# lucaspk512/vrdone

Measured on AMD Instinct MI355X. Metric: subject-object pairs/sec forward (2048 pairs x 256 frames x 512-d), higher is better.
Workload: dtype f16x3: f32 products as 3 scaled-f16 MFMA products (~22-bit), f32 accumulate; reference-grade: distance to a float64 run of the reference <= 1.4 x the reference's own float32 error (tests/golden/mask_vrd_f64.npz)

## Files before the change

### vrdone_amd/csrc/vrd_attn_x3.hip

```cpp
#include "vrd_common.h"
#include <cmath>
#include <cstdlib>
#include <type_traits>
#include <utility>

namespace {

using f32x16 = __attribute__((ext_vector_type(16))) float;
typedef __attribute__((ext_vector_type(8))) __bf16 bf16x8;
typedef __attribute__((ext_vector_type(4))) __bf16 bf16x4;
typedef __attribute__((ext_vector_type(4))) short s16x4;
typedef __attribute__((ext_vector_type(8))) short s16x8;
typedef __attribute__((address_space(3))) void* lds_ptr_t;
typedef __attribute__((address_space(3))) s16x4* lds_s16x4_ptr;

__device__ uint4 g_attn_zero[16];

template <int HD>
struct AG {
    static constexpr int ROWB = HD * 2;
    static constexpr int CPR = ROWB / 16;
    static constexpr int RPI = 1024 / ROWB;
    static constexpr int PLANE = 32 * ROWB;
    static constexpr int STAGE = 4 * PLANE;
// ... 251 lines not shown
__device__ __forceinline__ void split_pair(float p0, float p1, unsigned& hi, unsigned& lo) {
    if constexpr (F16) {
        typedef __attribute__((ext_vector_type(2))) _Float16 f16x2;
        const f16x2 h = {(_Float16)p0, (_Float16)p1};
        hi = __builtin_bit_cast(unsigned, h);
        const f16x2 l = {(_Float16)(p0 - (float)h[0]), (_Float16)(p1 - (float)h[1])};
        lo = __builtin_bit_cast(unsigned, l);
    } else {
        const bf16x2 h = {(__bf16)p0, (__bf16)p1};
        hi = __builtin_bit_cast(unsigned, h);
        const float h0 = __builtin_bit_cast(float, hi << 16), h1 = __builtin_bit_cast(float, hi & 0xffff0000u);
        const bf16x2 l = {(__bf16)(p0 - h0), (__bf16)(p1 - h1)};
        lo = __builtin_bit_cast(unsigned, l);
    }
}

#define VRD_MFMA(pre, ops, ...)                                                   \
    do {                                                                          \
        if constexpr (F16) asm volatile(pre "v_mfma_f32_32x32x16_f16 " ops __VA_ARGS__);  \
        else asm volatile(pre "v_mfma_f32_32x32x16_bf16 " ops __VA_ARGS__);       \
    } while (0)

template <int R0, int N>
__device__ __forceinline__ void agpr_scale(float alpha) {
    if constexpr (N > 0) {
        float t;
        asm volatile("v_accvgpr_read_b32 %0, a%c2\n\tv_mul_f32 %0, %0, %1\n\tv_accvgpr_write_b32 a%c2, %0"
                     : "=&v"(t) : "v"(alpha), "n"(R0));
        agpr_scale<R0 + 1, N - 1>(alpha);
    }
}

struct SmBlock {
    float x[16];
    float mx, mu, ae, alpha, sum;
    float mr, lp;
    u32x4 ph[2], pl[2];
};

#ifdef VRD_ATTN_STAMP
__device__ unsigned long long g_attn_stamp[65];
#define VRD_STAMP(i)                                                                      \
    do {                                                                                  \
        if (wave == 0) {                                                                  \
            unsigned long long t_;                                                        \
            asm volatile("s_memtime %0\n\ts_waitcnt lgkmcnt(0)" : "=s"(t_)::"memory");    \
            if (lane == 0) stamp_lds[i] = t_;                                             \
        }                                                                                 \
    } while (0)
#else
#define VRD_STAMP(i) do { } while (0)
#endif

template <int HD, bool F16, int NPROD = 3>
__global__ __launch_bounds__(256, 1) void attn_flash_x3_w64_kernel(const float* __restrict__ q, int64_t ldq,
                                                                  const float* __restrict__ k, const float* __restrict__ v,
                                                                  int64_t ldkv, const uint8_t* __restrict__ kv_mask,
                                                                  const uint8_t* __restrict__ q_mask, int Tq, int Tk, int width,
                                                                  float scale_log2e, float* __restrict__ out, int64_t ldo,
                                                                  int pair_out, int q_blocks, int n_head_, int n_batch, int prefetch, int item_step) {
    using G = AG<HD>;
    static_assert(NPROD == 3 || (NPROD == 1 && F16), "the one-product form exists for the f16 format only");
    constexpr bool LO = NPROD == 3;
    constexpr int KS = HD / 16;
    constexpr int DT = HD / 32;
    constexpr int NS = 4;
    constexpr int PER_WAVE = G::N_DMA / 4;
    constexpr int PPP = 32 / G::RPI;
    constexpr int NG_S = 6 * KS;
    constexpr int NG_O = 12 * DT;
    constexpr int HPG_S = 48 / NG_S, HPG_O = 48 / NG_O;
    constexpr int LEAD = 4;
#define VRD_AQ(qb, s) (8 * ((qb) * KS + (s)))
#define VRD_AO(qb, d) (128 + 16 * ((qb) * DT + (d)))
    static_assert(G::N_DMA % 4 == 0 && NG_S >= 24 && NG_O >= 24 && VRD_AQ(1, KS - 1) + 8 <= 128, "layout assumptions");
    extern __shared__ __attribute__((aligned(16))) float smem[];
    char* const lds = reinterpret_cast<char*>(smem);
    const int nkt = (Tk + 31) / 32, nqg = (Tq + 31) / 32;
    float* const kbias = reinterpret_cast<float*>(lds + NS * G::STAGE);
    int* const tile_on = reinterpret_cast<int*>(kbias + nkt * 32);
    int* const qgrp = tile_on + nkt;
    const int nk64 = (nkt * 32 + 63) & ~63, nq64 = (nqg * 32 + 63) & ~63;
    int* const raw_k = qgrp + nqg;
    int* const raw_q = raw_k + nk64;
#ifdef VRD_ATTN_STAMP
    unsigned long long* const stamp_lds = reinterpret_cast<unsigned long long*>(lds + 163840 - 64 * 8);
#endif

    const int tid = threadIdx.x, lane = tid & 63;
    const int wave = __builtin_amdgcn_readfirstlane(tid >> 6);
    const int li = lane & 31, lh = lane >> 5;
    const unsigned lds_base = (unsigned)reinterpret_cast<uintptr_t>((lds_ptr_t)lds);
    const int n_items = n_head_ * n_batch;
    bool masks_pending = true;
    auto fresh_lane = [&]() {
        int ln;
        asm volatile("v_mbcnt_lo_u32_b32 %0, -1, 0\n\tv_mbcnt_hi_u32_b32 %0, -1, %0" : "=v"(ln));
        return ln;
    };
    auto dma_masks = [&](int it2) {
        const int b2 = it2 / n_head_;
        const int ln = fresh_lane();
        if (kv_mask) {
            const uint8_t* base = kv_mask + (int64_t)b2 * Tk;
            for (int j = wave; j < nk64 / 64; j += 4) {
                const int key = j * 64 + ln;
                const unsigned voff = (unsigned)(key < Tk ? key : Tk - 1);
                const unsigned dst = lds_base + (unsigned)(reinterpret_cast<char*>(raw_k) - lds) + j * 256;
                asm volatile("s_mov_b32 m0, %0\n\ts_nop 0\n\tglobal_load_lds_ubyte %1, %2" ::"s"(dst), "v"(voff), "s"(base) : "memory");
            }
        }
        if (q_mask) {
            const uint8_t* base = q_mask + (int64_t)b2 * Tq;
            for (int j = wave; j < nq64 / 64; j += 4) {
                const int r = j * 64 + ln;
                const unsigned voff = (unsigned)(r < Tq ? r : Tq - 1);
                const unsigned dst = lds_base + (unsigned)(reinterpret_cast<char*>(raw_q) - lds) + j * 256;
                asm volatile("s_mov_b32 m0, %0\n\ts_nop 0\n\tglobal_load_lds_ubyte %1, %2" ::"s"(dst), "v"(voff), "s"(base) : "memory");
            }
        }
    };
    const int item_first = item_step == 1 ? (int)(((long long)n_items * blockIdx.x) / gridDim.x) : (int)blockIdx.x;
    const int item_end = item_step == 1 ? (int)(((long long)n_items * (blockIdx.x + 1)) / gridDim.x) : n_items;
    for (int item = item_first; item < item_end; item += item_step) {
    VRD_STAMP(0);
    const int h = item % n_head_, b = item / n_head_;
    if (prefetch && item == item_first) dma_masks(item);
    if (prefetch && masks_pending) asm volatile("s_waitcnt vmcnt(0)" ::: "memory");
    asm volatile("s_waitcnt lgkmcnt(0)" ::: "memory");
    __builtin_amdgcn_s_barrier();
    asm volatile("" ::: "memory");
    {
        const int ln = fresh_lane(), tn = wave * 64 + ln;
        for (int key = tn; key < nkt * 32; key += 256) {
            const bool ok = key < Tk && (!kv_mask || (prefetch ? raw_k[key] != 0 : kv_mask[(int64_t)b * Tk + (key < Tk ? key : Tk - 1)] != 0));
            kbias[key] = ok ? 0.f : -INFINITY;
            const unsigned long long bal = __ballot(ok);
            const unsigned bits = (unsigned)((bal >> (ln & 32)) & 0xffffffffull);
            if ((ln & 31) == 0) tile_on[key >> 5] = bits == 0u ? 0 : (bits == 0xffffffffu ? 2 : 1);
        }
        for (int r = tn; r < nqg * 32; r += 256) {
            const bool ok = r < Tq && (!q_mask || (prefetch ? raw_q[r] != 0 : q_mask[(int64_t)b * Tq + (r < Tq ? r : Tq - 1)] != 0));
            const unsigned long long bal = __ballot(ok);
            if ((ln & 31) == 0) qgrp[r >> 5] = ((bal >> (ln & 32)) & 0xffffffffull) != 0ull;
        }
    }
    asm volatile("s_waitcnt lgkmcnt(0)" ::: "memory");
    __builtin_amdgcn_s_barrier();
    asm volatile("" ::: "memory");
    if (prefetch && item + item_step < item_end) {
        dma_masks(item + item_step);
        masks_pending = true;
    }
    VRD_STAMP(1);
    for (int qblk = 0; qblk < q_blocks; ++qblk) {
    if (qblk) {
        asm volatile("s_waitcnt lgkmcnt(0)" ::: "memory");
        __builtin_amdgcn_s_barrier();
        asm volatile("" ::: "memory");
    }
    const int q0 = qblk * 256 + wave * 64;
    const char* kb = reinterpret_cast<const char*>(k + (int64_t)b * Tk * ldkv) + h * HD * 4;
    const char* vb = reinterpret_cast<const char*>(v + (int64_t)b * Tk * ldkv) + h * HD * 4;

    const int gq = qblk * 8 + (lane & 7);
    const unsigned blk_bits = (unsigned)(__ballot(gq < nqg && qgrp[gq < nqg ? gq : 0] != 0) & 0xffull);
    const bool live0 = (blk_bits >> (2 * wave)) & 1u, live1 = (blk_bits >> (2 * wave + 1)) & 1u;
    const bool q_live = live0 || live1;
    if (blk_bits == 0u) {
#ifndef VRD_ATTN_LAB_NOZERO
        {
            constexpr int LPRZ = HD / 4, RPIZ = 64 / LPRZ;
            const int row_end = Tq < qblk * 256 + 256 ? Tq : qblk * 256 + 256;
            const int ln = fresh_lane();
            int row = qblk * 256 + wave * RPIZ + ln / LPRZ;
            char* zp = reinterpret_cast<char*>(out + ((int64_t)b * Tq + row) * ldo) + h * HD * 4 + (ln % LPRZ) * 16;
            const int64_t zstep = ldo * 4 * (4 * RPIZ);
            const u32x4 zero4 = {0u, 0u, 0u, 0u};
#pragma unroll 1
            for (; row < row_end; row += 4 * RPIZ, zp += zstep) *reinterpret_cast<u32x4*>(zp) = zero4;
        }
#endif
        continue;
    }
    VRD_STAMP(55);
    asm volatile("" ::: VRD_ALL_AGPRS);
    {
        const char* qbase = reinterpret_cast<const char*>(q + (int64_t)b * Tq * ldq) + h * HD * 4;
        const int rin_q = lane / G::CPR, pch_q = lane % G::CPR;
        const unsigned qrowbytes = (unsigned)(ldq * 4);
        static_for<2 * PPP>([&](auto u_c) {
            constexpr int qb = decltype(u_c)::value / PPP, rb = decltype(u_c)::value % PPP;
            const int row = rb * G::RPI + rin_q;
            const int tq = q0 + 32 * qb + row;
            const int lc = pch_q ^ G::kswz(row);
            const unsigned voff = (unsigned)(tq < Tq ? tq : Tq - 1) * qrowbytes + (unsigned)((lc >> 2) * 128 + (lc & 3) * 16);
            const unsigned dst = lds_base + (2 * qb + (wave >> 1)) * G::STAGE + (wave & 1) * 2 * G::PLANE + rb * 1024;
            const char* const src_hi = qbase + 0;
            const char* const src_lo = src_hi + 64;
            asm volatile("s_mov_b32 m0, %0\n\ts_nop 0\n\tglobal_load_lds_dwordx4 %1, %2" ::"s"(dst), "v"(voff), "s"(src_hi) : "memory");
            asm volatile("s_mov_b32 m0, %0\n\ts_nop 0\n\tglobal_load_lds_dwordx4 %1, %2" ::"s"(dst + G::PLANE), "v"(voff), "s"(src_lo) : "memory");
        });
    }
    VRD_STAMP(56);
    static_for<2 * DT * 16>([&](auto r_c) {
        asm volatile("v_accvgpr_write_b32 a%c0, 0" :: "n"(128 + decltype(r_c)::value));
    });
    VRD_STAMP(57);

    const int rin = lane / G::CPR, pch = lane % G::CPR;
    const int row0 = (wave % PPP) * G::RPI + rin;
    const int rowbytes = (int)(ldkv * 4);
    auto chunk_of = [&](int row, bool is_v) {
        const int lc = pch ^ (is_v ? G::vswz(row) : G::kswz(row));
        return (lc >> 2) * 128 + (lc & 3) * 16;
    };
    constexpr int HALF_ROWS = HD == 128 ? 16 : 0;
    struct Req {
        const char *kbase, *vbase;
        unsigned vk[2], vv[2];
        int half;
    };
    auto req_of = [&](int kt) {
        Req r;
        if (kt * 32 + 32 <= Tk) {
            r.kbase = kb + (int64_t)kt * 32 * rowbytes;
            r.vbase = vb + (int64_t)kt * 32 * rowbytes;
            r.vk[0] = r.vk[1] = (unsigned)(row0 * rowbytes) + chunk_of(row0, false);
            r.vv[0] = r.vv[1] = (unsigned)(row0 * rowbytes) + chunk_of(row0, true);
            r.half = HALF_ROWS * rowbytes;
        } else {
            r.kbase = kb;
            r.vbase = vb;
#pragma unroll
            for (int u = 0; u < 2; ++u) {
                int key = kt * 32 + row0 + HALF_ROWS * u;
                key = key < Tk ? key : Tk - 1;
                r.vk[u] = (unsigned)(key * rowbytes) + chunk_of(row0, false);
                r.vv[u] = (unsigned)(key * rowbytes) + chunk_of(row0, true);
            }
            r.half = 0;
        }
        return r;
    };
    auto issue1 = [&](const Req& r, int buf, auto i_c) __attribute__((always_inline)) {
        constexpr int i = decltype(i_c)::value;
        constexpr int u = HD == 128 ? (i & 1) : 0;
        const int j = wave + 4 * i;
        const int plane = j / PPP, rb = j % PPP;
        const unsigned dst = lds_base + buf * G::STAGE + plane * G::PLANE + rb * 1024;
        const char* sbase = (plane < 2 ? r.kbase : r.vbase) + ((plane & 1) ? 64 : 0) + (u ? r.half : 0);
        const unsigned voff = plane < 2 ? r.vk[u] : r.vv[u];
        asm volatile("s_mov_b32 m0, %0\n\ts_nop 0\n\tglobal_load_lds_dwordx4 %1, %2" ::"s"(dst), "v"(voff), "s"(sbase) : "memory");
    };

    unsigned long long act = ~0ull;
    if (nkt <= 64) act = __ballot(lane < nkt && tile_on[lane < nkt ? lane : 0] != 0);
    auto next_on = [&](int from) {
        if (from >= nkt) return nkt;
        if (nkt > 64) return from;
        const unsigned long long m = act & (~0ull << from);
        return m ? (int)__builtin_ctzll(m) : nkt;
    };
    const int n_act = nkt <= 64 ? (int)__builtin_popcountll(act) : nkt;
    unsigned long long cln = 0ull;
    if (nkt <= 64) cln = __ballot(lane < nkt && tile_on[lane < nkt ? lane : 0] == 2);
    const int krow = li * G::ROWB;
    const int vq = (lane >> 2) & 3, vp = lane & 3;
    const int vcol0 = 16 * ((lane >> 4) & 1) + 4 * vp;

    struct KF { bf16x8 h, l; };
    auto load_k = [&](const char* st, int s) __attribute__((always_inline)) {
        KF f;
        const int off = krow + (((2 * s + lh) ^ G::kswz(li)) * 16);
        f.h = *reinterpret_cast<const bf16x8*>(st + off);
        if (LO) f.l = *reinterpret_cast<const bf16x8*>(st + G::PLANE + off);
        return f;
    };
    auto load_v = [&](const char* st, int s, int d) __attribute__((always_inline)) {
        KF f;
        s16x8 rh, rl;
#pragma unroll
        for (int part = 0; part < 2; ++part) {
            const int row = 16 * s + 8 * part + 4 * lh + vq;
            const int col = 32 * d + vcol0;
            const int off = row * G::ROWB + ((((col * 2) >> 4) ^ G::vswz(row)) * 16) + ((col * 2) & 15);
            const s16x4 th = __builtin_amdgcn_ds_read_tr16_b64_v4i16((lds_s16x4_ptr)(st + 2 * G::PLANE + off));
            s16x4 tl = th;
            if (LO) tl = __builtin_amdgcn_ds_read_tr16_b64_v4i16((lds_s16x4_ptr)(st + 3 * G::PLANE + off));
#pragma unroll
            for (int j = 0; j < 4; ++j) {
                rh[4 * part + j] = th[j];
                rl[4 * part + j] = tl[j];
            }
        }
        f.h = __builtin_bit_cast(bf16x8, rh);
        f.l = __builtin_bit_cast(bf16x8, rl);
        return f;
    };

    SmBlock A, B;
    A.mr = B.mr = -INFINITY;
    A.lp = B.lp = 0.f;
    float tsp[4];
    unsigned long long cmask[2] = {0ull, 0ull};
    const float thr = F16 ? 8.0f : 16.0f;
// ... 100 lines not shown
        } else if constexpr (i == 72) {
            float ta, tb;
            asm volatile("v_exp_f32 %2, %6\n\tv_exp_f32 %3, %7\n\tv_add_f32 %4, %8, %10\n\tv_add_f32 %5, %9, %11\n\t"
                         "v_fma_f32 %0, %0, %2, %4\n\tv_fma_f32 %1, %1, %3, %5"
                         : "+v"(A.lp), "+v"(B.lp), "=&v"(A.alpha), "=&v"(B.alpha), "=&v"(ta), "=&v"(tb)
                         : "v"(A.ae), "v"(B.ae), "v"(A.sum), "v"(B.sum), "v"(A.x[15]), "v"(B.x[15]));
        }
    };

    auto mfma_s = [&](auto s_c, auto j_c, const KF& kf, f32x16& sa, f32x16& sb) __attribute__((always_inline)) {
        constexpr int s = decltype(s_c)::value, j = decltype(j_c)::value, qb = j & 1;
        f32x16& acc = qb ? sb : sa;
        constexpr int aq = VRD_AQ(qb, s) + (j >= 2 && j < 4 ? 4 : 0);
        if constexpr (!LO) {
            if constexpr (j < 4) {
            } else if constexpr (s == 0)
                VRD_MFMA("", "%0, %1, a[%c2:%c3], 0", : "=&v"(acc) : "v"(kf.h), "n"(aq), "n"(aq + 3));
            else
                VRD_MFMA("", "%0, %1, a[%c2:%c3], %0", : "+v"(acc) : "v"(kf.h), "n"(aq), "n"(aq + 3));
        } else if constexpr (s == 0 && j < 2) {
            VRD_MFMA("", "%0, %1, a[%c2:%c3], 0", : "=&v"(acc) : "v"(kf.l), "n"(aq), "n"(aq + 3));
        } else if constexpr (j < 2) {
            VRD_MFMA("", "%0, %1, a[%c2:%c3], %0", : "+v"(acc) : "v"(kf.l), "n"(aq), "n"(aq + 3));
        } else {
            VRD_MFMA("", "%0, %1, a[%c2:%c3], %0", : "+v"(acc) : "v"(kf.h), "n"(aq), "n"(aq + 3));
        }
    };
    auto mfma_o = [&](auto g_c, auto j_c, const KF& vf) __attribute__((always_inline)) {
        constexpr int g = decltype(g_c)::value, j = decltype(j_c)::value, qb = j & 1, s = g / DT, d = g % DT;
        constexpr int ao = VRD_AO(qb, d);
        const SmBlock& X = qb ? B : A;
        if constexpr (!LO) {
            if constexpr (j < 4) {
            } else if constexpr (d == 0 && j == 4)
                VRD_MFMA("s_nop 1\n\t", "a[%c2:%c3], %0, %1, a[%c2:%c3]", :: "v"(vf.h), "v"(X.ph[s]), "n"(ao), "n"(ao + 15));
            else
                VRD_MFMA("", "a[%c2:%c3], %0, %1, a[%c2:%c3]", :: "v"(vf.h), "v"(X.ph[s]), "n"(ao), "n"(ao + 15));
        } else if constexpr (j < 2) {
            if constexpr (d == 0 && j == 0)
                VRD_MFMA("s_nop 1\n\t", "a[%c2:%c3], %0, %1, a[%c2:%c3]", :: "v"(vf.l), "v"(X.ph[s]), "n"(ao), "n"(ao + 15));
            else
                VRD_MFMA("", "a[%c2:%c3], %0, %1, a[%c2:%c3]", :: "v"(vf.l), "v"(X.ph[s]), "n"(ao), "n"(ao + 15));
        } else if constexpr (j < 4) {
            VRD_MFMA("", "a[%c2:%c3], %0, %1, a[%c2:%c3]", :: "v"(vf.h), "v"(X.pl[s]), "n"(ao), "n"(ao + 15));
        } else {
            VRD_MFMA("", "a[%c2:%c3], %0, %1, a[%c2:%c3]", :: "v"(vf.h), "v"(X.ph[s]), "n"(ao), "n"(ao + 15));
        }
    };
    auto rescale = [&](auto qb_c, float alpha) __attribute__((always_inline)) {
        agpr_scale<VRD_AO(decltype(qb_c)::value, 0), 16 * DT>(alpha);
    };

    auto tile = [&](auto with_s_c, f32x16& sa_c, f32x16& sb_c, f32x16& sa_n, f32x16& sb_n, const char* st,
                    const char* st1, const float* kbs, bool dirty, bool do_req, const Req& req, int buf_req, bool first) __attribute__((always_inline)) {
        constexpr bool WITH_S = decltype(with_s_c)::value;
        if (dirty) {
#pragma unroll
            for (int g = 0; g < 4; ++g) {
                const float4 bv = *reinterpret_cast<const float4*>(kbs + 8 * g + 4 * lh);
                sa_c[4 * g + 0] += bv.x;
                sa_c[4 * g + 1] += bv.y;
                sa_c[4 * g + 2] += bv.z;
                sa_c[4 * g + 3] += bv.w;
                sb_c[4 * g + 0] += bv.x;
                sb_c[4 * g + 1] += bv.y;
                sb_c[4 * g + 2] += bv.z;
                sb_c[4 * g + 3] += bv.w;
            }
        }
        KF kf{}, kn{}, vf{}, vn{};
        if (WITH_S) kf = load_k(st1, 0);
        VRD_SB();
        static_for<LEAD>([&](auto u_c) { sm_piece(u_c, sa_c, sb_c); });
        VRD_SB();
        static_for<KS>([&](auto s_c) {
            constexpr int s = decltype(s_c)::value;
            static_for<6>([&](auto j_c) {
                constexpr int j = decltype(j_c)::value, gap = 6 * s + j;
                if constexpr (WITH_S) mfma_s(s_c, j_c, kf, sa_n, sb_n);
                if constexpr (j == 0 && WITH_S && s + 1 < KS) kn = load_k(st1, s + 1);
                if constexpr (gap == NG_S - 4) vf = load_v(st, 0, 0);
                static_for<HPG_S>([&](auto u_c) {
                    constexpr int piece = LEAD + gap * HPG_S + decltype(u_c)::value;
                    if constexpr (piece < 48) sm_piece(ic<piece>{}, sa_c, sb_c);
                });
                VRD_SB();
            });
            kf = kn;
        });
        if (!first && cmask[0] != 0ull) rescale(ic<0>{}, __builtin_amdgcn_exp2f(A.ae));
        if (!first && cmask[1] != 0ull) rescale(ic<1>{}, __builtin_amdgcn_exp2f(B.ae));
        VRD_SB();
        static_for<2 * DT>([&](auto g_c) {
            constexpr int g = decltype(g_c)::value;
            static_for<6>([&](auto j_c) {
                constexpr int j = decltype(j_c)::value, gap = 6 * g + j;
                mfma_o(g_c, j_c, vf);
                if constexpr (j == 0 && g + 1 < 2 * DT) vn = load_v(st, (g + 1) / DT, (g + 1) % DT);
                static_for<HPG_O>([&](auto u_c) { sm_piece(ic<48 + gap * HPG_O + decltype(u_c)::value>{}, sa_c, sb_c); });
                constexpr int rq = gap - NG_O / 2 - 1;
                if constexpr (rq >= 0 && rq % 3 == 0 && rq / 3 < PER_WAVE) {
                    if (do_req) issue1(req, buf_req, ic<rq / 3>{});
                }
                VRD_SB();
            });
            vf = vn;
        });
    };

    int kt_iss = -1;
    int issued = 0;
    auto request_next = [&](int buf) {
        if (issued < n_act) {
            kt_iss = next_on(kt_iss + 1);
            const Req r = req_of(kt_iss);
            static_for<PER_WAVE>([&](auto i_c) { issue1(r, buf, i_c); });
            ++issued;
        }
    };
    VRD_STAMP(51);
    asm volatile("s_waitcnt vmcnt(0)" ::: "memory");
    masks_pending = false;
    VRD_STAMP(52);
    static_for<2>([&](auto qb_c) {
        constexpr int qb = decltype(qb_c)::value;
        static_for<KS>([&](auto s_c) {
            constexpr int s = decltype(s_c)::value;
            const char* stq = lds + (2 * qb + (wave >> 1)) * G::STAGE + (wave & 1) * 2 * G::PLANE;
            const int off = li * G::ROWB + (((2 * s + lh) ^ G::kswz(li)) * 16);
            const u32x4 th = *reinterpret_cast<const u32x4*>(stq + off), tl = *reinterpret_cast<const u32x4*>(stq + G::PLANE + off);
            constexpr int r = VRD_AQ(qb, s);
            asm volatile("v_accvgpr_write_b32 a%c8, %0\n\tv_accvgpr_write_b32 a%c9, %1\n\tv_accvgpr_write_b32 a%c10, %2\n\t"
                         "v_accvgpr_write_b32 a%c11, %3\n\tv_accvgpr_write_b32 a%c12, %4\n\tv_accvgpr_write_b32 a%c13, %5\n\t"
                         "v_accvgpr_write_b32 a%c14, %6\n\tv_accvgpr_write_b32 a%c15, %7"
                         :: "v"(th[0]), "v"(th[1]), "v"(th[2]), "v"(th[3]), "v"(tl[0]), "v"(tl[1]), "v"(tl[2]), "v"(tl[3]), "n"(r), "n"(r + 1),
                            "n"(r + 2), "n"(r + 3), "n"(r + 4), "n"(r + 5), "n"(r + 6), "n"(r + 7));
        });
        asm volatile("s_waitcnt lgkmcnt(0)" ::: "memory");
        __builtin_amdgcn_s_barrier();
        if constexpr (qb == 0) {
            request_next(0);
            request_next(1);
        } else {
            request_next(2);
        }
    });
    static_assert(NS == 4, "the prologue requests three tiles");
    VRD_STAMP(2);
    int kt_cur = next_on(0);
    f32x16 s0a, s0b, s1a, s1b;
#pragma unroll
    for (int e = 0; e < 16; ++e) s0a[e] = s0b[e] = s1a[e] = s1b[e] = 0.f;
    if (n_act > 0) {
        if (n_act >= 3) asm volatile("s_waitcnt vmcnt(%0)" ::"n"(2 * PER_WAVE) : "memory");
        else if (n_act == 2) asm volatile("s_waitcnt vmcnt(%0)" ::"n"(PER_WAVE) : "memory");
        else asm volatile("s_waitcnt vmcnt(0)" ::: "memory");
        __builtin_amdgcn_s_barrier();
        VRD_STAMP(54);
        if (q_live) {
            KF kf = load_k(lds, 0), kn = kf;
            static_for<KS>([&](auto s_c) {
                constexpr int s = decltype(s_c)::value;
                if constexpr (s + 1 < KS) kn = load_k(lds, s + 1);
                static_for<6>([&](auto j_c) { mfma_s(s_c, j_c, kf, s0a, s0b); });
                kf = kn;
            });
            asm volatile("s_nop 15" : "+v"(s0a), "+v"(s0b));
        }
    }
    VRD_STAMP(3);
    int it = 0;
    auto step = [&](f32x16& ca, f32x16& cb, f32x16& na, f32x16& nb) __attribute__((always_inline)) {
        const bool has_next = it + 1 < n_act;
        const int kt_next = has_next ? next_on(kt_cur + 1) : nkt;
        if (has_next) {
            if (it + 2 < issued) asm volatile("s_waitcnt vmcnt(%0)" ::"n"(PER_WAVE) : "memory");
            else asm volatile("s_waitcnt vmcnt(0)" ::: "memory");
        }
        VRD_STAMP(4 + 3 * it);
        __builtin_amdgcn_s_barrier();
        VRD_STAMP(5 + 3 * it);
        const bool do_req = issued < n_act;
        if (do_req) {
            kt_iss = next_on(kt_iss + 1);
            ++issued;
        }
        const Req req = req_of(do_req ? kt_iss : 0);
        const char* st = lds + (it & (NS - 1)) * G::STAGE;
        const char* st1 = lds + ((it + 1) & (NS - 1)) * G::STAGE;
        const float* kbs = kbias + kt_cur * 32;
        const int buf_req = (it + NS - 1) & (NS - 1);
        if (q_live) {
            const bool dirty = nkt <= 64 ? ((cln >> kt_cur) & 1ull) == 0ull : __builtin_amdgcn_readfirstlane(tile_on[kt_cur]) != 2;
            if (has_next) tile(std::true_type{}, ca, cb, na, nb, st, st1, kbs, dirty, do_req, req, buf_req, it == 0);
            else tile(std::false_type{}, ca, cb, na, nb, st, st1, kbs, dirty, do_req, req, buf_req, it == 0);
        } else if (do_req) {
            static_for<PER_WAVE>([&](auto i_c) { issue1(req, buf_req, i_c); });
        }
        kt_cur = kt_next;
        VRD_STAMP(6 + 3 * it);
        ++it;
    };
    while (it < n_act) {
        step(s0a, s0b, s1a, s1b);
        if (it >= n_act) break;
        step(s1a, s1b, s0a, s0b);
    }

    asm volatile("s_nop 15\n\ts_nop 15" ::: "memory");
    __builtin_amdgcn_s_barrier();
    VRD_STAMP(40);
    constexpr int CH = HD / 4;
    char* const slab = lds + wave * (64 * HD * 4);
    static_for<2>([&](auto qb_c) {
        constexpr int qb = decltype(qb_c)::value;
        const float l_tot = xchg32_sum(qb ? B.lp : A.lp);
        const float inv = (qb ? live1 : live0) ? ((F16 && !pair_out) ? vrd::F16_ACT_INV : 1.0f) / l_tot : 0.f;
        static_for<DT>([&](auto d_c) {
            constexpr int d = decltype(d_c)::value;
            static_for<4>([&](auto g_c) {
                constexpr int g = decltype(g_c)::value, r = VRD_AO(qb, d) + 4 * g;
                float4 val;
                asm volatile("v_accvgpr_read_b32 %0, a%c4\n\tv_accvgpr_read_b32 %1, a%c5\n\tv_accvgpr_read_b32 %2, a%c6\n\t"
                             "v_accvgpr_read_b32 %3, a%c7"
                             : "=v"(val.x), "=v"(val.y), "=v"(val.z), "=v"(val.w) : "n"(r), "n"(r + 1), "n"(r + 2), "n"(r + 3));
                val.x *= inv;
                val.y *= inv;
                val.z *= inv;
                val.w *= inv;
                const int c16 = 8 * d + 2 * g + lh;
                *reinterpret_cast<float4*>(slab + (32 * qb + li) * (HD * 4) + ((c16 ^ (li & (CH - 1))) * 16)) = val;
            });
        });
    });
    VRD_STAMP(41);
    const bool all_rows = q0 + 64 <= Tq;
    if (pair_out) {
        constexpr int LPR = CH / 2;
        constexpr int ROWS_PI = 64 / LPR;
        constexpr int NT = 64 / ROWS_PI, BATCH = 4;
        const int rr = lane / LPR, cj = lane % LPR;
        char* gp = reinterpret_cast<char*>(out + ((int64_t)b * Tq + (q0 + rr < Tq ? q0 + rr : Tq - 1)) * ldo) +
                   vrd::pair_index(h * HD + 8 * cj) * 2;
        const int64_t gstep = ldo * 4 * ROWS_PI;
#pragma unroll 1
        for (int t0 = 0; t0 < NT; t0 += BATCH) {
            float4 va[BATCH], vb[BATCH];
#pragma unroll
            for (int u = 0; u < BATCH; ++u) {
                const int r = (t0 + u) * ROWS_PI + rr;
                va[u] = *reinterpret_cast<const float4*>(slab + r * (HD * 4) + (((2 * cj) ^ (r & (CH - 1))) * 16));
                vb[u] = *reinterpret_cast<const float4*>(slab + r * (HD * 4) + (((2 * cj + 1) ^ (r & (CH - 1))) * 16));
            }
#pragma unroll
            for (int u = 0; u < BATCH; ++u) {
                const int r = (t0 + u) * ROWS_PI + rr;
                if (all_rows || q0 + r < Tq) {
                    uint4 hi, lo;
                    split_pair<F16>(va[u].x, va[u].y, hi.x, lo.x);
                    split_pair<F16>(va[u].z, va[u].w, hi.y, lo.y);
                    split_pair<F16>(vb[u].x, vb[u].y, hi.z, lo.z);
                    split_pair<F16>(vb[u].z, vb[u].w, hi.w, lo.w);
#ifndef VRD_ATTN_LAB_NOSTORE
                    *reinterpret_cast<uint4*>(gp) = hi;
                    *reinterpret_cast<uint4*>(gp + 64) = lo;
#else
                    asm volatile("" ::"v"(hi.x), "v"(hi.y), "v"(hi.z), "v"(hi.w), "v"(lo.x), "v"(lo.y), "v"(lo.z), "v"(lo.w));
#endif
                }
                gp += gstep;
            }
        }
    } else {
        constexpr int ROWS_PI = 64 / CH;
        constexpr int NT = 64 / ROWS_PI, BATCH = 8;
        const int rr = lane / CH, cj = lane % CH;
        char* gp = reinterpret_cast<char*>(out + ((int64_t)b * Tq + (q0 + rr < Tq ? q0 + rr : Tq - 1)) * ldo) + (h * HD + 4 * cj) * 4;
        const int64_t gstep = ldo * 4 * ROWS_PI;
#pragma unroll 1
        for (int t0 = 0; t0 < NT; t0 += BATCH) {
            float4 val[BATCH];
#pragma unroll
            for (int u = 0; u < BATCH; ++u) {
                const int r = (t0 + u) * ROWS_PI + rr;
                val[u] = *reinterpret_cast<const float4*>(slab + r * (HD * 4) + ((cj ^ (r & (CH - 1))) * 16));
            }
#pragma unroll
            for (int u = 0; u < BATCH; ++u) {
                const int r = (t0 + u) * ROWS_PI + rr;
                if (all_rows || q0 + r < Tq) *reinterpret_cast<float4*>(gp) = val[u];
                gp += gstep;
            }
        }
    }
    VRD_STAMP(42 + qblk);
    }
#ifdef VRD_ATTN_STAMP
    VRD_STAMP(50);
    if (blockIdx.x == 0 && wave == 0) {
        asm volatile("s_waitcnt lgkmcnt(0)" ::: "memory");
        g_attn_stamp[lane] += stamp_lds[lane] - stamp_lds[0];
        if (lane == 0) g_attn_stamp[64] += 1;
    }
#endif
    }
#undef VRD_AQ
#undef VRD_AO
#undef VRD_MFMA
}

template <int HD, bool F16, int NPROD = 3>
int launch_w64(const float* q, int64_t ldq, const float* k, const float* v, int64_t ldkv, const uint8_t* kv_mask, const uint8_t* q_mask, int B,
               int Tq, int Tk, int n_head, float scale, float* out, int64_t ldo, int pair_out, hipStream_t s) {
    auto kern = attn_flash_x3_w64_kernel<HD, F16, NPROD>;
    constexpr size_t lds_all = 160 * 1024;
    constexpr size_t lds_max = 4 * AG<HD>::STAGE + (4096 + 128 + 2048) * sizeof(float);
    const size_t nkt = (size_t)(Tk + 31) / 32, nqg = (size_t)(Tq + 31) / 32;
    const size_t lds_tables = 4 * AG<HD>::STAGE + (nkt * 33 + nqg) * sizeof(float);
    const size_t lds_staged = lds_tables + (((nkt * 32 + 63) & ~(size_t)63) + ((nqg * 32 + 63) & ~(size_t)63)) * sizeof(float);
    if (lds_tables > lds_max) {
        vrd::set_error("vrd_attention_pair: Tk = %d exceeds the 4096 keys the key-bias row is sized for", Tk);
        return -1;
    }
    const char* const pf_e = getenv("VRD_FLASH_PREFETCH");
    const int prefetch = (!pf_e || atoi(pf_e) != 0) && lds_staged <= lds_all;
    if (int rc = vrd::reserve_lds(reinterpret_cast<const void*>(kern), lds_all, "vrd_attention_pair(w64)")) return rc;
    const int q_blocks = (Tq + 255) / 256;
#ifdef VRD_ATTN_STAMP
    const size_t lds_launch = lds_all;
#else
    const size_t lds_launch = prefetch ? lds_staged : lds_tables;
#endif
    static const int n_cu = [] {
        int dev = 0, n = 256;
        if (hipGetDevice(&dev) == hipSuccess) (void)hipDeviceGetAttribute(&n, hipDeviceAttributeMultiprocessorCount, dev);
        return n > 0 ? n : 256;
    }();
    const int n_items = n_head * B;
    const char* const grid_e = getenv("VRD_FLASH_GRID");
    const int grid_cap = grid_e && atoi(grid_e) > 0 ? atoi(grid_e) : n_cu;
    const int grid = n_items < grid_cap ? n_items : grid_cap;
    const char* const walk_e = getenv("VRD_FLASH_WALK");
    const int item_step = walk_e && atoi(walk_e) == 0 ? grid : 1;
    hipLaunchKernelGGL(kern, dim3((unsigned)grid), dim3(256), lds_launch, s, q, ldq, k, v, ldkv, kv_mask, q_mask,
                       Tq, Tk, n_head * HD, scale * 1.44269504088896340736f, out, ldo, pair_out, q_blocks, n_head, B, prefetch, item_step);
    return 0;
}

template <int HD, int NW, bool F16, int NPROD = 3>
int launch(const float* q, int64_t ldq, const float* k, const float* v, int64_t ldkv, const uint8_t* kv_mask, const uint8_t* q_mask, int B, int Tq,
           int Tk, int n_head, float scale, float* out, int64_t ldo, int pair_out, hipStream_t s) {
    auto kern = attn_flash_x3_kernel<HD, NW, F16, NPROD>;
    constexpr size_t lds_max = 2 * AG<HD>::STAGE + (4096 + 128) * sizeof(float);
    const size_t lds = 2 * AG<HD>::STAGE + (size_t)((Tk + 31) / 32) * 33 * sizeof(float);
    if (lds > lds_max) {
        vrd::set_error("vrd_attention_pair: Tk = %d exceeds the 4096 keys the key-bias row is sized for", Tk);
        return -1;
    }
    if (int rc = vrd::reserve_lds(reinterpret_cast<const void*>(kern), lds_max, "vrd_attention_pair")) return rc;
    const int tiles = (Tq + 31) / 32;
    const int q_blocks = (tiles + NW - 1) / NW;
    hipLaunchKernelGGL(kern, dim3((unsigned)q_blocks * n_head * B), dim3(NW * 64), lds, s, q, ldq, k, v, ldkv, kv_mask, q_mask, Tq, Tk,
                       n_head * HD, scale, out, ldo, pair_out, q_blocks, n_head);
    return 0;
}

inline bool aligned16(const void* ptr) { return (reinterpret_cast<uintptr_t>(ptr) & 15u) == 0; }

}

#ifdef VRD_ATTN_STAMP
extern "C" int vrd_lab_attn_stamps(unsigned long long* dst65, int reset) {
    if (hipMemcpyFromSymbol(dst65, HIP_SYMBOL(g_attn_stamp), 65 * sizeof(unsigned long long)) != hipSuccess) return -1;
    if (reset) {
        unsigned long long z[65] = {};
        if (hipMemcpyToSymbol(HIP_SYMBOL(g_attn_stamp), z, sizeof(z)) != hipSuccess) return -1;
    }
    return 0;
}
#endif

extern "C" int vrd_attention_pair(const float* q, int64_t ldq, const float* k, const float* v, int64_t ldkv,
                                  const uint8_t* kv_mask, const uint8_t* q_mask, int B, int Tq, int Tk, int n_head, int head_dim,
                                  float* out, int64_t ldo, int out_pair, int pair_fmt, void* stream, int products) {
    VRD_CHECK_ARG(q && k && v && out, "vrd_attention_pair: null pointer");
    VRD_CHECK_ARG(head_dim == 64 || head_dim == 128, "vrd_attention_pair: head_dim must be 64 or 128 (got %d)", head_dim);
    VRD_CHECK_ARG(B > 0 && B <= 65535 && Tq > 0 && Tk > 0 && n_head > 0 && n_head <= 65535, "vrd_attention_pair: bad sizes");
    const int width = n_head * head_dim;
    VRD_CHECK_ARG(ldq >= width && ldkv >= width && ldo >= width && ldq % 4 == 0 && ldkv % 4 == 0 && ldo % 4 == 0 &&
                      aligned16(q) && aligned16(k) && aligned16(v) && aligned16(out),
                  "vrd_attention_pair: rows must be 16-byte aligned pair rows of width n_head*head_dim");
    VRD_CHECK_ARG(pair_fmt == VRD_PAIR_BF16 || pair_fmt == VRD_PAIR_F16, "vrd_attention_pair: pair_fmt must be VRD_PAIR_BF16 or VRD_PAIR_F16");
    VRD_CHECK_ARG(out_pair == VRD_PAIR_NONE || out_pair == pair_fmt, "vrd_attention_pair: pair output comes in the operands' format");
    VRD_CHECK_ARG(products == 0 || products == 3 || (products == 1 && pair_fmt == VRD_PAIR_F16),
                  "vrd_attention_pair: products must be 0 or 3, or 1 with VRD_PAIR_F16 operands (got %d, pair_fmt %d)", products, pair_fmt);
    hipStream_t s = static_cast<hipStream_t>(stream);
    const bool f16 = pair_fmt == VRD_PAIR_F16;
    const float scale = (f16 ? vrd::F16_ACT_INV * vrd::F16_ACT_INV : 1.0f) / sqrtf((float)head_dim);
// ... 26 lines not shown
```

Before: 15670.

## Prefetch next Q block into free stage slots during tile loop; move epilogue slab

Adds a lookahead path that finds the next live (item, q-block) and issues its Q loads into LDS stage buffers during the key-tile loop, using request slots that are otherwise idle. The following block then skips its own Q load and waits only on the outstanding count. The output epilogue is restructured to stage each 32-column chunk through a small per-wave slab at the top of LDS and store it immediately, so the prefetched Q stages are not overwritten. This hides the Q-load latency at block boundaries, but it adds more complex vmcnt bookkeeping and extra LDS use.

```diff
diff --git a/vrdone_amd/csrc/vrd_attn_x3.hip b/vrdone_amd/csrc/vrd_attn_x3.hip
--- a/vrdone_amd/csrc/vrd_attn_x3.hip
+++ b/vrdone_amd/csrc/vrd_attn_x3.hip
@@ -327,13 +327,16 @@
 #define VRD_STAMP(i) do { } while (0)
 #endif
 
+constexpr int W64_LDS_ALL = 160 * 1024, W64_SLAB_WAVE = 4096, W64_SLAB_OFF = W64_LDS_ALL - 512 - 4 * W64_SLAB_WAVE;
+
 template <int HD, bool F16, int NPROD = 3>
 __global__ __launch_bounds__(256, 1) void attn_flash_x3_w64_kernel(const float* __restrict__ q, int64_t ldq,
                                                                   const float* __restrict__ k, const float* __restrict__ v,
                                                                   int64_t ldkv, const uint8_t* __restrict__ kv_mask,
                                                                   const uint8_t* __restrict__ q_mask, int Tq, int Tk, int width,
                                                                   float scale_log2e, float* __restrict__ out, int64_t ldo,
-                                                                  int pair_out, int q_blocks, int n_head_, int n_batch, int prefetch, int item_step) {
+                                                                  int pair_out, int q_blocks, int n_head_, int n_batch, int prefetch, int item_step,
+                                                                  int lookahead) {
     using G = AG<HD>;
     static_assert(NPROD == 3 || (NPROD == 1 && F16), "the one-product form exists for the f16 format only");
     constexpr bool LO = NPROD == 3;
@@ -397,6 +400,17 @@
     };
     const int item_first = item_step == 1 ? (int)(((long long)n_items * blockIdx.x) / gridDim.x) : (int)blockIdx.x;
     const int item_end = item_step == 1 ? (int)(((long long)n_items * (blockIdx.x + 1)) / gridDim.x) : n_items;
+    int ah_item = -1, ah_blk = 0;
+    bool ah_counted = false;
+    auto q_piece = [&](const char* base, int row0, unsigned dst, int rb, int ln) __attribute__((always_inline)) {
+        const int row = rb * G::RPI + ln / G::CPR;
+        const int tq = row0 + row;
+        const int lc = (ln % G::CPR) ^ G::kswz(row);
+        const unsigned voff = (unsigned)(tq < Tq ? tq : Tq - 1) * (unsigned)(ldq * 4) + (unsigned)((lc >> 2) * 128 + (lc & 3) * 16);
+        asm volatile("s_mov_b32 m0, %0\n\ts_nop 0\n\tglobal_load_lds_dwordx4 %1, %2" ::"s"(dst), "v"(voff), "s"(base) : "memory");
+        const char* const base_lo = base + 64;
+        asm volatile("s_mov_b32 m0, %0\n\ts_nop 0\n\tglobal_load_lds_dwordx4 %1, %2" ::"s"(dst + G::PLANE), "v"(voff), "s"(base_lo) : "memory");
+    };
     for (int item = item_first; item < item_end; item += item_step) {
     VRD_STAMP(0);
     const int h = item % n_head_, b = item / n_head_;
@@ -442,7 +456,13 @@
     const unsigned blk_bits = (unsigned)(__ballot(gq < nqg && qgrp[gq < nqg ? gq : 0] != 0) & 0xffull);
     const bool live0 = (blk_bits >> (2 * wave)) & 1u, live1 = (blk_bits >> (2 * wave + 1)) & 1u;
     const bool q_live = live0 || live1;
+    const bool q_here = ah_item == item && ah_blk == qblk;
     if (blk_bits == 0u) {
+        if (q_here) {
+            asm volatile("s_waitcnt vmcnt(0)" ::: "memory");
+            masks_pending = false;
+            ah_item = -1;
+        }
 #ifndef VRD_ATTN_LAB_NOZERO
         {
             constexpr int LPRZ = HD / 4, RPIZ = 64 / LPRZ;
@@ -460,24 +480,30 @@
     }
     VRD_STAMP(55);
     asm volatile("" ::: VRD_ALL_AGPRS);
-    {
+    if (!q_here) {
         const char* qbase = reinterpret_cast<const char*>(q + (int64_t)b * Tq * ldq) + h * HD * 4;
-        const int rin_q = lane / G::CPR, pch_q = lane % G::CPR;
-        const unsigned qrowbytes = (unsigned)(ldq * 4);
         static_for<2 * PPP>([&](auto u_c) {
             constexpr int qb = decltype(u_c)::value / PPP, rb = decltype(u_c)::value % PPP;
-            const int row = rb * G::RPI + rin_q;
-            const int tq = q0 + 32 * qb + row;
-            const int lc = pch_q ^ G::kswz(row);
-            const unsigned voff = (unsigned)(tq < Tq ? tq : Tq - 1) * qrowbytes + (unsigned)((lc >> 2) * 128 + (lc & 3) * 16);
-            const unsigned dst = lds_base + (2 * qb + (wave >> 1)) * G::STAGE + (wave & 1) * 2 * G::PLANE + rb * 1024;
-            const char* const src_hi = qbase + 0;
-            const char* const src_lo = src_hi + 64;
-            asm volatile("s_mov_b32 m0, %0\n\ts_nop 0\n\tglobal_load_lds_dwordx4 %1, %2" ::"s"(dst), "v"(voff), "s"(src_hi) : "memory");
-            asm volatile("s_mov_b32 m0, %0\n\ts_nop 0\n\tglobal_load_lds_dwordx4 %1, %2" ::"s"(dst + G::PLANE), "v"(voff), "s"(src_lo) : "memory");
+            q_piece(qbase, q0 + 32 * qb, lds_base + (2 * qb + (wave >> 1)) * G::STAGE + (wave & 1) * 2 * G::PLANE + rb * 1024, rb, lane);
         });
     }
     VRD_STAMP(56);
+    int nx_item = item, nx_blk = qblk + 1;
+    if (lookahead) {
+        for (; nx_blk < q_blocks; ++nx_blk) {
+            const int gn = nx_blk * 8 + (lane & 7);
+            if ((__ballot(gn < nqg && qgrp[gn < nqg ? gn : 0] != 0) & 0xffull) != 0ull) break;
+        }
+        if (nx_blk >= q_blocks) {
+            nx_item = item + item_step;
+            nx_blk = 0;
+        }
+    }
+    const bool have_next = lookahead && nx_item < item_end;
+    const char* const qbase_n = reinterpret_cast<const char*>(q + (int64_t)(nx_item / n_head_) * Tq * ldq) + (nx_item % n_head_) * HD * 4;
+    const int q0_n = nx_blk * 256 + wave * 64;
+    int qa_done = 0;
+    int n_qa = 0;
     static_for<2 * DT * 16>([&](auto r_c) {
         asm volatile("v_accvgpr_write_b32 a%c0, 0" :: "n"(128 + decltype(r_c)::value));
     });
@@ -527,6 +553,10 @@
         const char* sbase = (plane < 2 ? r.kbase : r.vbase) + ((plane & 1) ? 64 : 0) + (u ? r.half : 0);
         const unsigned voff = plane < 2 ? r.vk[u] : r.vv[u];
         asm volatile("s_mov_b32 m0, %0\n\ts_nop 0\n\tglobal_load_lds_dwordx4 %1, %2" ::"s"(dst), "v"(voff), "s"(sbase) : "memory");
+    };
+    static_assert(PPP == PER_WAVE, "a quarter of Q has as many row blocks as a tile step has request slots");
+    auto qa_piece = [&](int stage, int rb) __attribute__((always_inline)) {
+        q_piece(qbase_n, q0_n + 32 * (stage >> 1), lds_base + stage * G::STAGE + (wave & 1) * 2 * G::PLANE + rb * 1024, rb, fresh_lane());
     };
 
     unsigned long long act = ~0ull;
@@ -733,7 +763,7 @@
     };
 
     auto tile = [&](auto with_s_c, f32x16& sa_c, f32x16& sb_c, f32x16& sa_n, f32x16& sb_n, const char* st,
-                    const char* st1, const float* kbs, bool dirty, bool do_req, const Req& req, int buf_req, bool first) __attribute__((always_inline)) {
+                    const char* st1, const float* kbs, bool dirty, bool do_req, const Req& req, int buf_req, bool first, bool do_qa) __attribute__((always_inline)) {
         constexpr bool WITH_S = decltype(with_s_c)::value;
         if (dirty) {
 #pragma unroll
@@ -782,6 +812,7 @@
                 constexpr int rq = gap - NG_O / 2 - 1;
                 if constexpr (rq >= 0 && rq % 3 == 0 && rq / 3 < PER_WAVE) {
                     if (do_req) issue1(req, buf_req, ic<rq / 3>{});
+                    else if (do_qa) qa_piece(buf_req, rq / 3);
                 }
                 VRD_SB();
             });
@@ -800,8 +831,13 @@
         }
     };
     VRD_STAMP(51);
-    asm volatile("s_waitcnt vmcnt(0)" ::: "memory");
-    masks_pending = false;
+    if (q_here && ah_counted) {
+        asm volatile("s_waitcnt vmcnt(%0)" ::"n"(8 * DT) : "memory");
+    } else {
+        asm volatile("s_waitcnt vmcnt(0)" ::: "memory");
+        masks_pending = false;
+    }
+    ah_item = -1;
     VRD_STAMP(52);
     static_for<2>([&](auto qb_c) {
         constexpr int qb = decltype(qb_c)::value;
@@ -836,6 +872,7 @@
         if (n_act >= 3) asm volatile("s_waitcnt vmcnt(%0)" ::"n"(2 * PER_WAVE) : "memory");
         else if (n_act == 2) asm volatile("s_waitcnt vmcnt(%0)" ::"n"(PER_WAVE) : "memory");
         else asm volatile("s_waitcnt vmcnt(0)" ::: "memory");
+        masks_pending = false;
         __builtin_amdgcn_s_barrier();
         VRD_STAMP(54);
         if (q_live) {
@@ -856,7 +893,9 @@
         const int kt_next = has_next ? next_on(kt_cur + 1) : nkt;
         if (has_next) {
             if (it + 2 < issued) asm volatile("s_waitcnt vmcnt(%0)" ::"n"(PER_WAVE) : "memory");
-            else asm volatile("s_waitcnt vmcnt(0)" ::: "memory");
+            else if (n_qa == 0) asm volatile("s_waitcnt vmcnt(0)" ::: "memory");
+            else if (n_qa == 2 * PPP) asm volatile("s_waitcnt vmcnt(%0)" ::"n"(2 * PPP) : "memory");
+            else asm volatile("s_waitcnt vmcnt(%0)" ::"n"(4 * PPP) : "memory");
         }
         VRD_STAMP(4 + 3 * it);
         __builtin_amdgcn_s_barrier();
@@ -871,12 +910,19 @@
         const char* st1 = lds + ((it + 1) & (NS - 1)) * G::STAGE;
         const float* kbs = kbias + kt_cur * 32;
         const int buf_req = (it + NS - 1) & (NS - 1);
+        const bool do_qa = have_next && !do_req && (wave >> 1) == (buf_req & 1);
+        if (do_qa) {
+            qa_done |= 1 << (buf_req >> 1);
+            n_qa += 2 * PPP;
+        }
         if (q_live) {
             const bool dirty = nkt <= 64 ? ((cln >> kt_cur) & 1ull) == 0ull : __builtin_amdgcn_readfirstlane(tile_on[kt_cur]) != 2;
-            if (has_next) tile(std::true_type{}, ca, cb, na, nb, st, st1, kbs, dirty, do_req, req, buf_req, it == 0);
-            else tile(std::false_type{}, ca, cb, na, nb, st, st1, kbs, dirty, do_req, req, buf_req, it == 0);
+            if (has_next) tile(std::true_type{}, ca, cb, na, nb, st, st1, kbs, dirty, do_req, req, buf_req, it == 0, do_qa);
+            else tile(std::false_type{}, ca, cb, na, nb, st, st1, kbs, dirty, do_req, req, buf_req, it == 0, do_qa);
         } else if (do_req) {
             static_for<PER_WAVE>([&](auto i_c) { issue1(req, buf_req, i_c); });
+        } else if (do_qa) {
+            static_for<PPP>([&](auto i_c) { qa_piece(buf_req, decltype(i_c)::value); });
         }
         kt_cur = kt_next;
         VRD_STAMP(6 + 3 * it);
@@ -891,8 +937,28 @@
     asm volatile("s_nop 15\n\ts_nop 15" ::: "memory");
     __builtin_amdgcn_s_barrier();
     VRD_STAMP(40);
-    constexpr int CH = HD / 4;
-    char* const slab = lds + wave * (64 * HD * 4);
+    if (have_next) {
+        static_for<2>([&](auto qb_c) {
+            constexpr int qb = decltype(qb_c)::value;
+            if (!(qa_done & (1 << qb))) {
+                const int ln = fresh_lane();
+                static_for<PPP>([&](auto i_c) {
+                    constexpr int rb = decltype(i_c)::value;
+                    q_piece(qbase_n, q0_n + 32 * qb, lds_base + (2 * qb + (wave >> 1)) * G::STAGE + (wave & 1) * 2 * G::PLANE + rb * 1024, rb, ln);
+                });
+            }
+        });
+        ah_item = nx_item;
+        ah_blk = nx_blk;
+    }
+    VRD_STAMP(58);
+    const bool all_rows = q0 + 64 <= Tq;
+#ifndef VRD_ATTN_LAB_NOSTORE
+    ah_counted = all_rows;
+#else
+    ah_counted = false;
+#endif
+    char* const slab = lds + (lookahead ? W64_SLAB_OFF : 0) + wave * W64_SLAB_WAVE;
     static_for<2>([&](auto qb_c) {
         constexpr int qb = decltype(qb_c)::value;
         const float l_tot = xchg32_sum(qb ? B.lp : A.lp);
@@ -909,71 +975,45 @@
                 val.y *= inv;
                 val.z *= inv;
                 val.w *= inv;
-                const int c16 = 8 * d + 2 * g + lh;
-                *reinterpret_cast<float4*>(slab + (32 * qb + li) * (HD * 4) + ((c16 ^ (li & (CH - 1))) * 16)) = val;
+                *reinterpret_cast<float4*>(slab + li * 128 + (((2 * g + lh) ^ (li & 7)) * 16)) = val;
             });
+            if (pair_out) {
+                const int rr = lane >> 2, cj = lane & 3;
+                char* gp = reinterpret_cast<char*>(out + ((int64_t)b * Tq + q0 + 32 * qb + rr) * ldo) + vrd::pair_index(h * HD + 32 * d + 8 * cj) * 2;
+                auto rd = [&](int r, int c) { return *reinterpret_cast<const float4*>(slab + r * 128 + ((c ^ (r & 7)) * 16)); };
+                const float4 va0 = rd(rr, 2 * cj), vb0 = rd(rr, 2 * cj + 1), va1 = rd(16 + rr, 2 * cj), vb1 = rd(16 + rr, 2 * cj + 1);
+                auto st = [&](const float4& va, const float4& vb, int u) {
+                    if (all_rows || q0 + 32 * qb + 16 * u + rr < Tq) {
+                        uint4 hi, lo;
+                        split_pair<F16>(va.x, va.y, hi.x, lo.x);
+                        split_pair<F16>(va.z, va.w, hi.y, lo.y);
+                        split_pair<F16>(vb.x, vb.y, hi.z, lo.z);
+                        split_pair<F16>(vb.z, vb.w, hi.w, lo.w);
+#ifndef VRD_ATTN_LAB_NOSTORE
+                        *reinterpret_cast<uint4*>(gp + (int64_t)u * (ldo * 4 * 16)) = hi;
+                        *reinterpret_cast<uint4*>(gp + (int64_t)u * (ldo * 4 * 16) + 64) = lo;
+#else
+                        asm volatile("" ::"v"(hi.x), "v"(hi.y), "v"(hi.z), "v"(hi.w), "v"(lo.x), "v"(lo.y), "v"(lo.z), "v"(lo.w));
+#endif
+                    }
+                };
+                st(va0, vb0, 0);
+                st(va1, vb1, 1);
+            } else {
+                const int rr = lane >> 3, cj = lane & 7;
+                char* gp = reinterpret_cast<char*>(out + ((int64_t)b * Tq + q0 + 32 * qb + rr) * ldo) + (h * HD + 32 * d + 4 * cj) * 4;
+                auto rd = [&](int r) { return *reinterpret_cast<const float4*>(slab + r * 128 + ((cj ^ (r & 7)) * 16)); };
+                const float4 v0 = rd(rr), v1 = rd(8 + rr), v2 = rd(16 + rr), v3 = rd(24 + rr);
+                auto st = [&](const float4& val, int u) {
+                    if (all_rows || q0 + 32 * qb + 8 * u + rr < Tq) *reinterpret_cast<float4*>(gp + (int64_t)u * (ldo * 4 * 8)) = val;
+                };
+                st(v0, 0);
+                st(v1, 1);
+                st(v2, 2);
+                st(v3, 3);
+            }
         });
     });
-    VRD_STAMP(41);
-    const bool all_rows = q0 + 64 <= Tq;
-    if (pair_out) {
-        constexpr int LPR = CH / 2;
-        constexpr int ROWS_PI = 64 / LPR;
-        constexpr int NT = 64 / ROWS_PI, BATCH = 4;
-        const int rr = lane / LPR, cj = lane % LPR;
-        char* gp = reinterpret_cast<char*>(out + ((int64_t)b * Tq + (q0 + rr < Tq ? q0 + rr : Tq - 1)) * ldo) +
-                   vrd::pair_index(h * HD + 8 * cj) * 2;
-        const int64_t gstep = ldo * 4 * ROWS_PI;
-#pragma unroll 1
-        for (int t0 = 0; t0 < NT; t0 += BATCH) {
-            float4 va[BATCH], vb[BATCH];
-#pragma unroll
-            for (int u = 0; u < BATCH; ++u) {
-                const int r = (t0 + u) * ROWS_PI + rr;
-                va[u] = *reinterpret_cast<const float4*>(slab + r * (HD * 4) + (((2 * cj) ^ (r & (CH - 1))) * 16));
-                vb[u] = *reinterpret_cast<const float4*>(slab + r * (HD * 4) + (((2 * cj + 1) ^ (r & (CH - 1))) * 16));
-            }
-#pragma unroll
-            for (int u = 0; u < BATCH; ++u) {
-                const int r = (t0 + u) * ROWS_PI + rr;
-                if (all_rows || q0 + r < Tq) {
-                    uint4 hi, lo;
-                    split_pair<F16>(va[u].x, va[u].y, hi.x, lo.x);
-                    split_pair<F16>(va[u].z, va[u].w, hi.y, lo.y);
-                    split_pair<F16>(vb[u].x, vb[u].y, hi.z, lo.z);
-                    split_pair<F16>(vb[u].z, vb[u].w, hi.w, lo.w);
-#ifndef VRD_ATTN_LAB_NOSTORE
-                    *reinterpret_cast<uint4*>(gp) = hi;
-                    *reinterpret_cast<uint4*>(gp + 64) = lo;
-#else
-                    asm volatile("" ::"v"(hi.x), "v"(hi.y), "v"(hi.z), "v"(hi.w), "v"(lo.x), "v"(lo.y), "v"(lo.z), "v"(lo.w));
-#endif
-                }
-                gp += gstep;
-            }
-        }
-    } else {
-        constexpr int ROWS_PI = 64 / CH;
-        constexpr int NT = 64 / ROWS_PI, BATCH = 8;
-        const int rr = lane / CH, cj = lane % CH;
-        char* gp = reinterpret_cast<char*>(out + ((int64_t)b * Tq + (q0 + rr < Tq ? q0 + rr : Tq - 1)) * ldo) + (h * HD + 4 * cj) * 4;
-        const int64_t gstep = ldo * 4 * ROWS_PI;
-#pragma unroll 1
-        for (int t0 = 0; t0 < NT; t0 += BATCH) {
-            float4 val[BATCH];
-#pragma unroll
-            for (int u = 0; u < BATCH; ++u) {
-                const int r = (t0 + u) * ROWS_PI + rr;
-                val[u] = *reinterpret_cast<const float4*>(slab + r * (HD * 4) + ((cj ^ (r & (CH - 1))) * 16));
-            }
-#pragma unroll
-            for (int u = 0; u < BATCH; ++u) {
-                const int r = (t0 + u) * ROWS_PI + rr;
-                if (all_rows || q0 + r < Tq) *reinterpret_cast<float4*>(gp) = val[u];
-                gp += gstep;
-            }
-        }
-    }
     VRD_STAMP(42 + qblk);
     }
 #ifdef VRD_ATTN_STAMP
@@ -994,7 +1034,7 @@
 int launch_w64(const float* q, int64_t ldq, const float* k, const float* v, int64_t ldkv, const uint8_t* kv_mask, const uint8_t* q_mask, int B,
                int Tq, int Tk, int n_head, float scale, float* out, int64_t ldo, int pair_out, hipStream_t s) {
     auto kern = attn_flash_x3_w64_kernel<HD, F16, NPROD>;
-    constexpr size_t lds_all = 160 * 1024;
+    constexpr size_t lds_all = W64_LDS_ALL;
     constexpr size_t lds_max = 4 * AG<HD>::STAGE + (4096 + 128 + 2048) * sizeof(float);
     const size_t nkt = (size_t)(Tk + 31) / 32, nqg = (size_t)(Tq + 31) / 32;
     const size_t lds_tables = 4 * AG<HD>::STAGE + (nkt * 33 + nqg) * sizeof(float);
@@ -1005,12 +1045,14 @@
     }
     const char* const pf_e = getenv("VRD_FLASH_PREFETCH");
     const int prefetch = (!pf_e || atoi(pf_e) != 0) && lds_staged <= lds_all;
+    const char* const la_e = getenv("VRD_FLASH_AHEAD");
+    const int lookahead = prefetch && (!la_e || atoi(la_e) != 0) && lds_staged <= (size_t)W64_SLAB_OFF;
     if (int rc = vrd::reserve_lds(reinterpret_cast<const void*>(kern), lds_all, "vrd_attention_pair(w64)")) return rc;
     const int q_blocks = (Tq + 255) / 256;
 #ifdef VRD_ATTN_STAMP
     const size_t lds_launch = lds_all;
 #else
-    const size_t lds_launch = prefetch ? lds_staged : lds_tables;
+    const size_t lds_launch = lookahead ? (size_t)W64_SLAB_OFF + 4 * W64_SLAB_WAVE : (prefetch ? lds_staged : lds_tables);
 #endif
     static const int n_cu = [] {
         int dev = 0, n = 256;
@@ -1024,7 +1066,7 @@
     const char* const walk_e = getenv("VRD_FLASH_WALK");
     const int item_step = walk_e && atoi(walk_e) == 0 ? grid : 1;
     hipLaunchKernelGGL(kern, dim3((unsigned)grid), dim3(256), lds_launch, s, q, ldq, k, v, ldkv, kv_mask, q_mask,
-                       Tq, Tk, n_head * HD, scale * 1.44269504088896340736f, out, ldo, pair_out, q_blocks, n_head, B, prefetch, item_step);
+                       Tq, Tk, n_head * HD, scale * 1.44269504088896340736f, out, ldo, pair_out, q_blocks, n_head, B, prefetch, item_step, lookahead);
     return 0;
 }
 
```

New measurement: 15630. About the same (-0.2%).
